# soberguo/HOIGen

Hardware: AMD Instinct MI355X
Metric: union-crop embeddings/sec ViT-B/16 bs=256 (higher is better)
Workload: dtype f16; 1 GPU; CLIP ViT-B/16 union-region encode (encode_image), 224x224 crops, batch 256 per GPU, synthetic N(0,1) crops + seeded synthetic weights (BASELINE.json configs[1]); last_block=all rows (option last_block_row0 = 0), batch_per_gpu=256, global_batch=256, parallelism=dp1

## Files before the change

### hoigen_amd/_lib.py

```python
from __future__ import annotations

import ctypes as C
import os
import subprocess
import threading
from typing import Dict, Optional

HERE = os.path.dirname(os.path.abspath(__file__))
LIB_PATH = os.environ.get("HG_LIB_PATH") or os.path.join(HERE, "csrc", "libhoigen_amd.so")
HG_MAX_SLOTS = 16
HG_F32, HG_F16 = 0, 1


class hg_tensor(C.Structure):
    _fields_ = [("ptr", C.c_void_p), ("dtype", C.c_int32)]


_BLOCK_FIELDS = ["in_proj_weight", "in_proj_bias", "out_proj_weight", "out_proj_bias", "ln_1_weight",
                 "ln_1_bias", "c_fc_weight", "c_fc_bias", "c_proj_weight", "c_proj_bias", "ln_2_weight",
                 "ln_2_bias"]


class hg_block_weights(C.Structure):
    _fields_ = [(n, hg_tensor) for n in _BLOCK_FIELDS]
# ... 81 lines not shown
    "hg_assemble_prompts": (_I, [_P, _P, _P, _P, _P, _P, _I, _I, _I, _I, _I, _P, _P]),
    "hg_l2_normalize": (_I, [_P, _P, _I, _I, _P, _P]),
    "hg_vae_loss": (_I, [_P, _P, _P, _P, _P, _I, _I, _P, _P]),
    "hg_roi_align": (_I, [_P, _P, _I, _I, _I, _P, _I, C.c_float, _I, _P, _P, _P]),
    "hg_load_cache": (_I, [_P, _I, _P]),
    "hg_cache_logits": (_I, [_P, _I, _P, _I, _P, _P]),
    "hg_preprocess_crops": (_I, [_P, _P, _I, _I, _P, _I, _I, _I, C.c_uint32, _P, _P, _P]),
    "hg_workspace_bytes": (_I, [_P, C.POINTER(C.c_uint64)]),
    "hg_set_option": (_I, [_P, C.c_char_p, _I]),
    "hg_get_option": (_I, [_P, C.c_char_p, C.POINTER(C.c_int32)]),
    "hg_test_gemm": (_I, [_P, _P, _P, _P, _P, _I, _I, _I, _I, _I, _P]),
    "hg_test_gemm_ln": (_I, [_P, _P, _P, _P, _P, _I, _I, _I, _I, _I, _P, _P, _P, _P, _P, _P, _P, _P]),
    "hg_test_attention": (_I, [_P, _P, _P, _P, _I, _I, _I, _I, _P, _P]),
    "hg_test_qkv_attn": (_I, [_P, _P, _P, _P, _P, _P, _I, _I, _I, _I, _P, _P]),
    "hg_test_gemm_hilo": (_I, [_P, _P, _P, _P, _P, _I, _I, _I, _I, _I, _P, _P, _P, _P]),
    "hg_test_image_stream": (_I, [_P, _P, _I, _P, _P, _P]),
    "hg_test_text_stream": (_I, [_P, _P, _I, _I, _I, _P, _P, _P]),
    "hg_profile_begin": (_I, [_P, _I, _I]),
    "hg_profile_end": (_I, [_P, _P, _I, C.POINTER(C.c_int32)]),
}

_lib = None
_lock = threading.RLock()
_ctxs: Dict[int, int] = {}


def build(force: bool = False) -> str:
    script = os.path.join(HERE, "csrc", "build.sh")
    if force:
        for f in os.listdir(os.path.join(HERE, "csrc")):
# ... 82 lines not shown
```

### hoigen_amd/csrc/hg_api.hip

```cpp
#include <math.h>
#include <stdarg.h>
#include <stdio.h>
#include <stdlib.h>
#include <string.h>

#include <string>
#include <vector>

#include <algorithm>
#include <mutex>

#include "../../include/hoigen_amd.h"
#include "hg_kernels.h"

using namespace hg;

namespace {

struct Buf {
    void* p = nullptr;
    size_t bytes = 0;
};

struct BlockW {
// ... 99 lines not shown
    int opt_row0 = 1;
    int opt_ln_fuse = 1;
    int opt_adapter_fuse = 1;
    int opt_adapter_fold = 1;
    int opt_stream_hilo = 1;
    int opt_qkv_attn = 1;
    int opt_qkv_attn_min_seq = 32;
    int opt_qkv_attn_gsz = 0;
    int opt_text_ln_fold = 1;
    int opt_qkv_attn_c = 1;
    int opt_vae_fused = 1;
    int opt_mlp_pair = 1;
    int opt_mlp_pair_chunk = 32;
    int opt_mlp_pair_fc_slots = 32;
    int opt_mlp_pair_fault = 0;
    int n_cu = 256;
    int32_t* pair_err = nullptr;
    int32_t* range_flag = nullptr;
    int32_t* eot_flag = nullptr;
    int32_t* eot_flag_dev = nullptr;
    int prof_kind = HG_PROF_OFF;
    std::vector<hipEvent_t> prof_ev;
    std::vector<hg_prof_rec> prof_rec;
    size_t prof_n = 0;
};

namespace {

int fail(hg_ctx* c, int code, const char* fmt, ...) {
    char tmp[512];
// ... 558 lines not shown
    half_t* const hg = gs ? (half_t*)c->hg.p : nullptr;
    half_t* a_ln = gs ? hg : h;
    auto gs_args = [&](GemmArgs& g, const float* gamma) {
        if (!gs) return;
        g.gamma = gamma;
        if (g.hl == 1 || g.hl == 2) { g.out3 = hg; g.ld3 = D; a_ln = hg; }
        else a_ln = h;
    };
    const int pair_panels = (int)rup(mlp_pair_ready_words(M), 64);
    const bool pair_on = fuse && !adapters && c->opt_mlp_pair && c->pair_err && blocks.size() > 1;
    if (pair_on) {
        int rc = ensure(c, c->pair_ready, blocks.size() * (size_t)pair_panels * 4);
        if (rc) return rc;
        HG_HIP(hipMemsetAsync(c->pair_ready.p, 0, blocks.size() * (size_t)pair_panels * 4, s));
    }
    int rln_i = 0;
    bool x_is_hilo = false;
    auto rln_args = [&](GemmArgs& g) {
        if (!hilo) return;
        g.hl = rln_i == 0 ? 1 : (rln_i == n_rln - 1 ? 3 : 2);
        g.lo = (half_t*)c->xlo.p; g.muc = muc;
        x_is_hilo = g.hl != 3;
        ++rln_i;
    };
    for (size_t i = 0; i < blocks.size(); ++i) {
        const BlockW& b = blocks[i];
        const int kcat = kmode[i];
        if (adapters && c->vit.adapters.size() > i && c->vit.adapters[i].present) {
            const AdapterW& aw = c->vit.adapters[i];
            if (kcat) {
// ... 74 lines not shown
            g.lda = D + 64; g.K = D + 64; g.W = c->vit.adapters[i].fold[ac->priors ? 0 : 1].wk_out;
        }
        if (fuse) {
            g.out2 = h; g.stats = stats; g.stats_ld = sld; g.mu = mu;
            if (hilo_c) { g.out2 = att; g.ld2 = D + 64; }
            if (!kcat || hilo_c) rln_args(g);
            gs_args(g, b.ln2_w);
            HG_HIP(gemm(c, EPI_RESID_LN_F32, g, s));
            HG_HIP(launch_finalize_stats(stats, mr, mu, M, sld, 64, s, muc, false, c->range_flag));
        } else {
            HG_HIP(gemm(c, EPI_BIAS_RESID_F32, g, s));
        }
        g = GemmArgs{};
        g.A = h; g.lda = D; g.out = fc; g.ldc = 4 * D; g.M = M; g.N = 4 * D; g.K = D;
        GemmArgs pq{};
        bool pq_built = false, paired = false;
        if (fuse) {
            g.W = b.wf_fc; g.bias = b.bf_fc; g.cs = b.cs_fc; g.mr = mr;
            if (hilo_c) { g.A = att; g.lda = D + 64; }
            if (gs) { g.A = a_ln; g.W = b.w_fc; g.cs = b.csg_fc; }
            if (pair_on && i + 1 < blocks.size()) {
                pq.A = fc; pq.lda = 4 * D; pq.W = b.w_proj; pq.bias = b.b_proj; pq.out = x; pq.ldc = D; pq.M = M; pq.N = D; pq.K = 4 * D;
                pq.out2 = h_of(i + 1); pq.ld2 = ldh_of(i + 1); pq.stats = stats; pq.stats_ld = sld; pq.mu = mu;
                rln_args(pq);
                gs_args(pq, blocks[i + 1].ln1_w);
                pq_built = true;
                if (mlp_pair_ok(g, pq, c->n_cu)) {
                    PairGateScope gate(c->device, s);
                    ProfScope ps(c, s, HG_PROF_MLP_PAIR, M, 4 * D, D);
                    HG_HIP(launch_mlp_pair(g, pq, (unsigned*)c->pair_ready.p + i * (size_t)pair_panels, c->pair_err,
                                           c->opt_mlp_pair_chunk, c->opt_mlp_pair_fc_slots, c->n_cu, s, c->opt_mlp_pair_fault));
                    paired = true;
                }
            }
            if (!paired) HG_HIP(gemm(c, EPI_LN_BIAS_QGELU_F16, g, s));
        } else {
            HG_HIP(launch_layernorm_f16(x, b.ln2_w, b.ln2_b, h, M, D, nullptr, 0, 1, s));
            g.W = b.w_fc; g.bias = b.b_fc;
            HG_HIP(gemm(c, EPI_BIAS_QGELU_F16, g, s));
        }
        g = GemmArgs{};
        g.A = fc; g.lda = 4 * D; g.W = b.w_proj; g.bias = b.b_proj; g.out = x; g.ldc = D; g.M = M; g.N = D; g.K = 4 * D;
        if (fuse && i + 1 < blocks.size()) {
            if (pq_built) {
                g = pq;
            } else {
                g.out2 = h_of(i + 1); g.ld2 = ldh_of(i + 1); g.stats = stats; g.stats_ld = sld; g.mu = mu;
                rln_args(g);
                gs_args(g, blocks[i + 1].ln1_w);
            }
            if (!paired) HG_HIP(gemm(c, EPI_RESID_LN_F32, g, s));
            HG_HIP(launch_finalize_stats(stats, mr, mu, M, sld, 64, s, muc, false, c->range_flag));
        } else {
            HG_HIP(gemm(c, EPI_BIAS_RESID_F32, g, s));
        }
        if (trace) {
            float* tr = trace + (size_t)(i + 1) * trace_stride;
            if (x_is_hilo) HG_HIP(launch_copy_rows_hilo(h, (const half_t*)c->xlo.p, muc, tr, tr_rows, tr_stride, D, s));
            else HG_HIP(launch_copy_rows(x, tr, tr_rows, tr_stride, D, s));
        }
    }
    return HG_OK;
}

int ensure_tower_ws(hg_ctx* c, int M, int D) {
    const size_t Mp = rup(M, 256);
// ... 100 lines not shown
        if (hipDeviceGetAttribute(&ncu, hipDeviceAttributeMultiprocessorCount, device) == hipSuccess && ncu > 0) c->n_cu = ncu;
        if (hipHostMalloc((void**)&c->eot_flag, 64, hipHostMallocMapped) == hipSuccess && c->eot_flag) *c->eot_flag = 0;
        else c->eot_flag = nullptr;
        if (hipMalloc((void**)&c->eot_flag_dev, 64) != hipSuccess) c->eot_flag_dev = nullptr;
        else (void)hipMemset(c->eot_flag_dev, 0, 64);
        if (hipHostMalloc((void**)&c->pair_err, 64, hipHostMallocMapped) == hipSuccess && c->pair_err) *c->pair_err = 0;
        else c->pair_err = nullptr;
        if (hipHostMalloc((void**)&c->range_flag, 64, hipHostMallocMapped) == hipSuccess && c->range_flag) *c->range_flag = 0;
        else c->range_flag = nullptr;
    }
    struct { const char* env; const char* key; } init[] = {{"HG_CHUNK_ROWS", "chunk_rows"}, {"HG_LAST_BLOCK_ROW0", "last_block_row0"},
                                                           {"HG_LN_FUSE", "ln_fuse"}, {"HG_ADAPTER_FUSE", "adapter_fuse"},
                                                           {"HG_ADAPTER_FOLD", "adapter_fold"}, {"HG_STREAM_HILO", "stream_hilo"},
                                                           {"HG_QKV_ATTN", "qkv_attn"}, {"HG_QKV_ATTN_MIN_SEQ", "qkv_attn_min_seq"},
                                                           {"HG_QKV_ATTN_GSZ", "qkv_attn_gsz"}, {"HG_QKV_ATTN_C", "qkv_attn_c"}, {"HG_TEXT_LN_FOLD", "text_ln_fold"}, {"HG_VAE_FUSED", "vae_fused"},
                                                           {"HG_MLP_PAIR", "mlp_pair"},
                                                           {"HG_MLP_PAIR_CHUNK", "mlp_pair_chunk"}, {"HG_MLP_PAIR_FC_SLOTS", "mlp_pair_fc_slots"},
                                                           {"HG_MLP_PAIR_FAULT", "mlp_pair_fault"}};
    for (auto& o : init)
        if (const char* e = getenv(o.env)) (void)hg_set_option(c, o.key, atoi(e));
    c->err.clear();
    return c;
}

int hg_set_option(hg_ctx* c, const char* key, int value) {
    if (!c || !key) return HG_ERR_INVALID;
    const std::string k(key);
    if (k == "chunk_rows") {
        if (value < 256) return fail(c, HG_ERR_INVALID, "chunk_rows must be >= 256");
        c->max_chunk_rows = value;
    } else if (k == "last_block_row0") c->opt_row0 = value != 0;
// ... 11 lines not shown
        if (value < 0 || value > 6) return fail(c, HG_ERR_INVALID, "qkv_attn_gsz must be 0 .. 6 (got %d)", value);
        c->opt_qkv_attn_gsz = value;
    } else if (k == "text_ln_fold") {
        if (value < 0 || value > 2) return fail(c, HG_ERR_INVALID, "text_ln_fold must be 0, 1 or 2 (got %d)", value);
        c->opt_text_ln_fold = value;
    } else if (k == "qkv_attn_c") {
        if (value < 0 || value > 1) return fail(c, HG_ERR_INVALID, "qkv_attn_c must be 0 or 1 (got %d)", value);
        c->opt_qkv_attn_c = value;
    }
    else if (k == "vae_fused") {
        if (value < 0 || value > 2) return fail(c, HG_ERR_INVALID, "vae_fused must be 0, 1 or 2 (got %d)", value);
        c->opt_vae_fused = value;
    } else if (k == "mlp_pair") {
        if (value < 0 || value > 1) return fail(c, HG_ERR_INVALID, "mlp_pair must be 0 or 1 (got %d)", value);
        c->opt_mlp_pair = value;
    } else if (k == "mlp_pair_chunk") {
        if (value < 1 || value > 64) return fail(c, HG_ERR_INVALID, "mlp_pair_chunk must be 1 .. 64 (got %d)", value);
        c->opt_mlp_pair_chunk = value;
    } else if (k == "mlp_pair_fc_slots") {
        if (value < 1 || value > 64) return fail(c, HG_ERR_INVALID, "mlp_pair_fc_slots must be 1 .. 64 (got %d)", value);
        c->opt_mlp_pair_fc_slots = value;
    } else if (k == "mlp_pair_fault") {
        if (value < 0 || value > 1) return fail(c, HG_ERR_INVALID, "mlp_pair_fault must be 0 or 1 (got %d)", value);
        c->opt_mlp_pair_fault = value;
    }
    else return fail(c, HG_ERR_INVALID, "unknown option '%s'", key);
    return HG_OK;
}

int hg_get_option(hg_ctx* c, const char* key, int* value) {
// ... 1 lines not shown
    const std::string k(key);
    if (k == "chunk_rows") *value = c->max_chunk_rows;
    else if (k == "last_block_row0") *value = c->opt_row0;
    else if (k == "ln_fuse") *value = c->opt_ln_fuse;
    else if (k == "adapter_fuse") *value = c->opt_adapter_fuse;
    else if (k == "adapter_fold") *value = c->opt_adapter_fold;
    else if (k == "stream_hilo") *value = c->opt_stream_hilo;
    else if (k == "stream_lo_bits") *value = 8;
    else if (k == "qkv_attn") *value = c->opt_qkv_attn;
    else if (k == "qkv_attn_min_seq") *value = c->opt_qkv_attn_min_seq;
    else if (k == "qkv_attn_gsz") *value = c->opt_qkv_attn_gsz;
    else if (k == "qkv_attn_c") *value = c->opt_qkv_attn_c;
    else if (k == "text_ln_fold") *value = c->opt_text_ln_fold;
    else if (k == "vae_fused") *value = c->opt_vae_fused;
    else if (k == "mlp_pair") *value = c->opt_mlp_pair;
    else if (k == "mlp_pair_chunk") *value = c->opt_mlp_pair_chunk;
    else if (k == "mlp_pair_fc_slots") *value = c->opt_mlp_pair_fc_slots;
    else if (k == "mlp_pair_fault") *value = c->opt_mlp_pair_fault;
    else return fail(c, HG_ERR_INVALID, "unknown option '%s'", key);
    return HG_OK;
}

void hg_destroy(hg_ctx* c) {
    if (!c) return;
    DevGuard dev_guard_(c);
    (void)hipDeviceSynchronize();
    free_all(c->vit.owned);
    free_all(c->vit.owned_adapters);
    free_all(c->text.owned);
    for (auto& v : c->vae) free_all(v.owned);
// ... 193 lines not shown
    g.A = (half_t*)c->h.p; g.lda = K; g.W = (half_t*)c->att.p; g.bias = bias; g.M = M; g.N = N; g.K = K; g.ldc = N;
    g.out = x; g.out2 = (half_t*)c->qkv.p; g.stats = (float*)c->stats.p; g.stats_ld = sld; g.mu = (const float*)c->mu.p;
    g.lo = (half_t*)c->xlo.p; g.muc = (const float*)c->muc.p;
    if (!gemm_ring2_ok(g)) return fail(c, HG_ERR_INVALID, "hg_test_gemm_hilo: shape not eligible for gemm_ring2");
    for (int i = 0; i < steps; ++i) {
        g.hl = (hilo && steps >= 2) ? (i == 0 ? 1 : (i == steps - 1 ? 3 : 2)) : 0;
        ProfScope ps(c, s, EPI_RESID_LN_F32, M, N, K);
        hipError_t e = launch_gemm_ring2(EPI_RESID_LN_F32, g, s);
        ps.finish();
        if (e != hipSuccess) return fail(c, HG_ERR_HIP, "test gemm (hi / lo) launch failed: %s", hipGetErrorString(e));
        HG_HIP(launch_finalize_stats((const float*)c->stats.p, (float*)c->mr.p, (float*)c->mu.p, M, sld, 64, s, (float*)c->muc.p));
    }
    if (out2) HG_HIP(launch_f16_to_f32((const half_t*)c->qkv.p, out2, (size_t)M * N, s));
    if (mr_out) HG_HIP(hipMemcpyAsync(mr_out, c->mr.p, (size_t)M * 2 * 4, hipMemcpyDeviceToDevice, s));
    HG_HIP(hipMemcpyAsync(mu, c->mu.p, (size_t)M * 4, hipMemcpyDeviceToDevice, s));
    return HG_OK;
}

int hg_test_attention(hg_ctx* c, const float* qkv, const float* q0, const int32_t* sel, int n_seq, int L, int heads,
                      int causal, float* out, void* stream) {
    if (!c || !qkv || !out || n_seq <= 0 || L < 1 || L > ATTN_LONG_MAX_L || heads < 1) return HG_ERR_INVALID;
    hipStream_t s = (hipStream_t)stream;
    HG_ON_DEVICE(c);
    const int D = heads * 64;
    const size_t M = (size_t)n_seq * L;
    int rc = ensure(c, c->qkv, rup(M, 256) * 3 * D * 2);
    if (!rc) rc = ensure(c, c->att, rup(M, 256) * D * 2);
    if (!rc && q0) rc = ensure(c, c->cq, rup(n_seq, 256) * (size_t)D * 2);
    if (rc) return rc;
    HG_HIP(launch_f32_to_f16(qkv, (half_t*)c->qkv.p, M * 3 * D, s));
// ... 852 lines not shown
```

### hoigen_amd/csrc/hg_gemm_ring.hip

```cpp
#include <stdio.h>
#include <stdlib.h>

#include "hg_gemm_ring_body.h"

namespace hg {

template <int MF, int EPI, bool PH2>
__global__ __launch_bounds__(512, 2) void gemm_ring(const GemmArgs p, const int tiles_n, const int n_tiles,
                                                    const unsigned a_bytes, const int mode, const int gsz) {
#if defined(__HIP_DEVICE_COMPILE__)
    const RingTileList sc(n_tiles, tiles_n, gsz);
    if (sc.n_items() <= 0) return;
    gemm_ring_body<MF, EPI, PH2>(p, a_bytes, mode, sc);
#endif
}

template <int MF, int EPI, bool PH2 = false>
static hipError_t launch_ring_t(const GemmArgs& a_in, hipStream_t s) {
    GemmArgs a = a_in;
    if (!a.ld2) a.ld2 = a.ldc;
    constexpr int BM = 64 * MF;
    constexpr int RING = 2 * (2 * MF * 4096 + 2 * 16384);
    constexpr bool LNC = (EPI == EPI_LN_BIAS_F16 || EPI == EPI_LN_BIAS_QGELU_F16);
    const int LDS = RING + a.N * 4 * (LNC ? 2 : 1) + (LNC ? BM * 8 : 0);
    if (LDS > 160 * 1024) return hipErrorInvalidValue;
    static bool attr_set_d[HG_MAX_DEVICES] = {};
    static int n_cu_d[HG_MAX_DEVICES];
    const int dev_i = current_device_index();
    bool& attr_set = attr_set_d[dev_i];
    int& n_cu = n_cu_d[dev_i];
    if (!attr_set) {
        n_cu = 256;
        hipError_t e = hipFuncSetAttribute(reinterpret_cast<const void*>(&gemm_ring<MF, EPI, PH2>),
                                           hipFuncAttributeMaxDynamicSharedMemorySize, 160 * 1024);
        if (e != hipSuccess) return e;
        int dev = 0;
        hipDeviceProp_t prop;
        if (hipGetDevice(&dev) == hipSuccess && hipGetDeviceProperties(&prop, dev) == hipSuccess)
            n_cu = prop.multiProcessorCount;
        attr_set = true;
    }
    const int tiles_m = (a.M + BM - 1) / BM, tiles_n = a.N / 256;
    const int n_tiles = tiles_m * tiles_n;
    int grid = n_tiles < n_cu ? n_tiles : n_cu;
    if (MF == 4 && n_tiles > n_cu) {
        const int rounds = (n_tiles + n_cu - 1) / n_cu;
        const int g8 = (((n_tiles + rounds - 1) / rounds) + 7) & ~7;
        if (g8 < grid) grid = g8;
// ... 3 lines not shown
    int gsz = (int)((1536 * 1024) / ((size_t)512 * a.K));
    if (gsz < 3) gsz = 3;
    if (gsz > tiles_n) gsz = tiles_n;
    {
        const int ngroups = (tiles_n + gsz - 1) / gsz;
        gsz = (tiles_n + ngroups - 1) / ngroups;
    }
#ifdef HG_STAMPS
    if (getenv("HG_STAMPS")) {
        const size_t n = (size_t)grid * 8 * 16;
        unsigned long long* d = nullptr;
        if (hipMalloc(&d, n * 8) != hipSuccess) return hipErrorOutOfMemory;
        hipMemsetAsync(d, 0, n * 8, s);
        GemmArgs b = a;
        b.dbg = d;
        hipLaunchKernelGGL((gemm_ring<MF, EPI, PH2>), dim3(grid), dim3(512), LDS, s, b, tiles_n, n_tiles, (unsigned)a_bytes, mode, gsz);
        hipStreamSynchronize(s);
        unsigned long long* h = (unsigned long long*)malloc(n * 8);
        hipMemcpy(h, d, n * 8, hipMemcpyDeviceToHost);
        static const char* names[8] = {"vmcnt", "lgkmcnt", "fetch-barrier", "MFMA", "mfma-barrier", "DMA-issue", "ds_read-issue", "epilogue"};
        for (int w = 0; w < 8; w += 4) {
            double acc[10] = {0};
            for (int blk = 0; blk < grid; ++blk)
                for (int k = 0; k < 10; ++k) acc[k] += (double)h[(size_t)(blk * 8 + w) * 16 + k];
            const double kts = acc[9] > 0 ? acc[9] : 1;
            fprintf(stderr, "[stamps] ring<%d,%d> N=%d K=%d wave %d: loop %.0f cycles/K-tile;", MF, EPI, a.N, a.K, w, acc[8] / kts);
            for (int k = 0; k < 8; ++k)
                if ((HG_STAMP_MASK >> k) & 1) fprintf(stderr, " %s %.0f", names[k], acc[k] / kts);
            fprintf(stderr, "\n");
        }
        free(h);
        hipFree(d);
        return hipGetLastError();
    }
#endif
    hipLaunchKernelGGL((gemm_ring<MF, EPI, PH2>), dim3(grid), dim3(512), LDS, s, a, tiles_n, n_tiles, (unsigned)a_bytes, mode, gsz);
    return hipGetLastError();
}

bool gemm_ring_ok(const GemmArgs& a) {
    if (a.N % 256 || a.K % 64 || a.K < 256 || a.M < 512 || a.N > 8192) return false;
    const size_t Mp = (size_t)((a.M + 255) / 256) * 256;
    if (Mp * a.lda * 2 >= (1ull << 31) || (size_t)a.N * a.K * 2 >= (1ull << 31)) return false;
    return true;
}

bool gemm_ln_ok(int epi, const GemmArgs& a) {
    if (!gemm_ring_ok(a)) return false;
    if (epi == EPI_RESID_LN_F32) return gemm_ring2_ok(a) && a.out2 && a.stats && a.mu && a.stats_ld == 4 * (a.N / 256);
    return a.cs && a.mr && a.N <= 3584;
}
// ... 22 lines not shown
        HG_RING(EPI_BIAS_QGELU_F16);
        HG_RING(EPI_BIAS_RELU_F16);
        HG_RING(EPI_BIAS_RESID_F32);
        HG_RING(EPI_BIAS_F32);
        HG_RING(EPI_PATCH_F32);
        HG_RING(EPI_BIAS_RELU_F32);
        HG_RING(EPI_SCALE_RESID_F32);
        HG_RING(EPI_LN_BIAS_F16);
        HG_RING(EPI_LN_BIAS_QGELU_F16);
        case EPI_RESID_LN_F32: return launch_ring_t<4, EPI_RESID_LN_F32, false>(a, s);
        default: return hipErrorInvalidValue;
    }
#undef HG_RING
}

}
```

### hoigen_amd/csrc/hg_gemm_ring_body.h

```cpp
#pragma once
#include <type_traits>

#include "hg_gemm_dev.h"

namespace hg {

#ifdef HG_STAMPS
#ifndef HG_STAMP_MASK
#define HG_STAMP_MASK 0xFF
#endif
#define SEG_B(k) do { if constexpr ((HG_STAMP_MASK >> (k)) & 1) t_beg = __builtin_amdgcn_s_memtime(); } while (0)
#define SEG_E(k) do { if constexpr ((HG_STAMP_MASK >> (k)) & 1) tacc[k] += __builtin_amdgcn_s_memtime() - t_beg; } while (0)
#else
#define SEG_B(k) do {} while (0)
#define SEG_E(k) do {} while (0)
#endif

template <int MF, int EPI, bool PH2, class SCHED>
__device__ __forceinline__ void gemm_ring_body(const GemmArgs& p, const unsigned a_bytes, const int mode, const SCHED& sc) {
#if defined(__HIP_DEVICE_COMPILE__)
    constexpr int BM = 64 * MF, BK = 64;
    constexpr int AH = MF * 4096, BH = 16384;
    constexpr int STAGE = 2 * AH + 2 * BH;
    constexpr int GA = MF / 2, GB = 2;
    static_assert(GA <= 2, "DMA piece helpers cover two pieces per half-tile");
    constexpr int N1 = 2 * GA + 3 * GB, N2 = 3 * GA + 2 * GB;
    constexpr bool RLN = (EPI == EPI_RESID_LN_F32);
    constexpr bool RESID = (EPI == EPI_BIAS_RESID_F32 || EPI == EPI_SCALE_RESID_F32 || RLN);
    constexpr bool F16_STORES = (EPI == EPI_BIAS_F16 || EPI == EPI_BIAS_QGELU_F16 || EPI == EPI_BIAS_RELU_F16 ||
                                 EPI == EPI_LN_BIAS_F16 || EPI == EPI_LN_BIAS_QGELU_F16);
    constexpr int E_RAW = RLN ? 8 * MF + 4 * MF + 2 * MF : (F16_STORES ? 4 * MF : 8 * MF);
    constexpr int E = E_RAW > 52 ? 52 : E_RAW;
    constexpr bool XPRE = RESID && MF == 2;
    constexpr bool LNC = (EPI == EPI_LN_BIAS_F16 || EPI == EPI_LN_BIAS_QGELU_F16);
    constexpr bool ROLL = RESID && MF == 4;
    constexpr int ROLL_W = RLN ? 6 : 8;
    constexpr int R = XPRE ? E : (ROLL ? ROLL_W + (RLN ? 1 : 0) : 0);
    constexpr bool PUB = SCHED::PUBLISH;
    static_assert(!PUB || (PH2 && (EPI == EPI_LN_BIAS_F16 || EPI == EPI_LN_BIAS_QGELU_F16)), "hand-off: two-phase loop, fp16 LayerNorm-fold epilogues");
    constexpr int BIAS_OFF = 2 * STAGE;
    const int MR_OFF = BIAS_OFF + 2 * p.N * 4;
    extern __shared__ __attribute__((aligned(16))) char smem[];
#ifdef HG_STAMPS
    unsigned long long tacc[8] = {0, 0, 0, 0, 0, 0, 0, 0}, t_beg = 0, t_all = 0;
#endif
    const int tid = sc.thread_id(), lane = tid & 63;
    const int wave = __builtin_amdgcn_readfirstlane(tid >> 6);
    const int wm = wave >> 2, wn = wave & 3;
    const int nk = p.K / BK;

    const int bid = blockIdx.x;
    const int n_items = sc.n_items();
// ... 186 lines not shown
    int g = 0;
    bool prev_full = false;
    int tm_prev = 0;
    (void)tm_prev;
    for (int r = 0; r < n_items; ++r) {
        int tm, tn, kb_r, ke_r;
        item_get(r, tm, tn, kb_r, ke_r);
        const int klen = nk;
        const int m0 = tm * BM, n0 = tn * 256;
        const bool post_ok = prev_full;
        prev_full = m0 + BM <= p.M;
        zero_acc();
        f32x4 xres[XPRE ? 2 : 1][XPRE ? 2 : 1][XPRE ? MF : 1][XPRE ? 2 : 1];
        f32x4 xw[ROLL ? ROLL_W : 1];
        float muw[RLN ? 2 : 1];
        auto chunk_row = [&](int rg) {
            int m = m0 + (rg / MF) * (BM / 2) + wm * MF * 16 + (rg % MF) * 16 + (lane & 15);
            return m < p.M ? m : p.M - 1;
        };
        auto chunk_load = [&](int c) {
            const int rg = c >> 2, hb = (c >> 1) & 1, g2 = c & 1;
            const int n = n0 + hb * 128 + wn * 32 + g2 * 16 + 4 * (lane >> 4);
            return *reinterpret_cast<const f32x4*>(reinterpret_cast<const float*>(p.out) + (size_t)chunk_row(rg) * p.ldc + n);
        };
        auto ph2_ktile = [&](auto KIND_T) {
            constexpr int KINDX = decltype(KIND_T)::value;
            constexpr int KIND = KINDX >= 4 ? 0 : KINDX;
            const int buf = (g & 1) * STAGE;
            const bool post = post_ok;
            const bool more = KIND < 2 || r + 1 < n_items;
// ... 72 lines not shown
            ph2_ktile(K1{});
            if constexpr (PUB) {
                ph2_ktile(std::integral_constant<int, 4>{});
                ph2_ktile(std::integral_constant<int, 5>{});
            }
            for (int kt = PUB ? 3 : 1; kt < klen - 2; ++kt) {
                ph2_ktile(K0{});
            }
            ph2_ktile(K2{});
            ph2_ktile(K3{});
        } else {
        for (int kt = 0; kt < klen; ++kt, ++g) {
            const int buf = (g & 1) * STAGE;
            const bool more = g + 2 < S;
            const bool post = post_ok;
            const bool xl = (XPRE || ROLL) && kt == klen - 1;
            read_A(0, buf);
            read_W(I0{}, buf);
            if constexpr (LNC) {
                if (kt == klen - 2 && lane < BM / 16)
                    __builtin_amdgcn_raw_ptr_buffer_load_lds(rsM, (HG_LDS void*)(smem + MR_OFF + wave * BM), 16, lane * 16,
                                                             (m0 + wave * (BM / 8)) * 8, 0, 0);
            }
            if (g + 1 < S) issue_A(1, 0, GA);
            if constexpr (ROLL) {
                if (xl) {
#pragma unroll
                    for (int c = 0; c < ROLL_W; ++c) xw[c] = chunk_load(c);
                    if constexpr (RLN) muw[0] = p.mu[chunk_row(0)];
                }
            }
            if constexpr (XPRE) {
                if (xl) {
#pragma unroll
                    for (int ha = 0; ha < 2; ++ha)
#pragma unroll
                        for (int f = 0; f < MF; ++f) {
                            int m = m0 + ha * (BM / 2) + wm * MF * 16 + f * 16 + (lane & 15);
                            m = m < p.M ? m : p.M - 1;
#pragma unroll
                            for (int hb = 0; hb < 2; ++hb)
#pragma unroll
                                for (int g2 = 0; g2 < 2; ++g2) {
                                    const int n = n0 + hb * 128 + wn * 32 + g2 * 16 + 4 * (lane >> 4);
                                    xres[ha][hb][f][g2] = *reinterpret_cast<const f32x4*>(
// ... 89 lines not shown
                    u32x4 st0, st1;
#pragma unroll
                    for (int j = 0; j < 4; ++j) {
                        const unsigned send = low ? d[4 + j] : d[j];
                        const unsigned recv = (unsigned)__builtin_amdgcn_update_dpp(0, (int)send, 0x128, 0xF, 0xF, false);
                        st0[j] = low ? d[j] : recv;
                        st1[j] = low ? recv : d[4 + j];
                    }
                    const int row0 = mb + (r16 & 7);
                    if (INTERIOR || row0 < p.M) *reinterpret_cast<u32x4*>(colp + (size_t)row0 * p.ldc) = st0;
                    if (INTERIOR || row0 + 8 < p.M) *reinterpret_cast<u32x4*>(colp + (size_t)(row0 + 8) * p.ldc) = st1;
                }
            };
            if (m0 + BM <= p.M) f16_epilogue(std::true_type{});
            else f16_epilogue(std::false_type{});
        } else if constexpr (ROLL) {
            const int q = lane >> 4;
            typedef unsigned u32x2 __attribute__((ext_vector_type(2)));
            typedef unsigned u32x4 __attribute__((ext_vector_type(4)));
#pragma unroll
            for (int rg = 0; rg < 2 * MF; ++rg) {
                const int ha = rg / MF, f = rg % MF;
                const int m = m0 + ha * (BM / 2) + wm * MF * 16 + f * 16 + (lane & 15);
                f32x4 v[2][2];
                float mu_r = 0.f;
                if constexpr (RLN) {
                    mu_r = muw[rg & 1];
                    if (rg + 1 < 2 * MF) muw[(rg + 1) & 1] = p.mu[chunk_row(rg + 1)];
                }
#pragma unroll
// ... 103 lines not shown
```

### hoigen_amd/csrc/hg_kernels.h

```cpp
#pragma once
#include <hip/hip_runtime.h>
#include <stdint.h>

#include "hg_common.h"

namespace hg {

enum Epilogue : int {
    EPI_BIAS_F16 = 0,
    EPI_BIAS_QGELU_F16 = 1,
    EPI_BIAS_RELU_F16 = 2,
    EPI_BIAS_RESID_F32 = 3,
    EPI_BIAS_F32 = 4,
    EPI_PATCH_F32 = 5,
    EPI_BIAS_RELU_F32 = 6,
    EPI_SCALE_RESID_F32 = 7,
    EPI_LN_BIAS_F16 = 8,
    EPI_LN_BIAS_QGELU_F16 = 9,
    EPI_RESID_LN_F32 = 10,
    EPI_MU_BIAS_RELU_F32 = 11,
    EPI_SCALE_RESID_LN_F32 = 12
};

#ifndef HG_LO_SCALE
// ... 24 lines not shown
    const float* muc = nullptr;
    const float* gamma = nullptr;
    half_t* out3 = nullptr;
    int ld3 = 0;
};
inline size_t gemm_lo_bytes(int M, int N) { return (size_t)((M + 127) / 128) * (N / 256) * 65536; }

hipError_t launch_gemm(int epi, const GemmArgs& a, hipStream_t s);
double gemm_flops(const GemmArgs& a);
bool gemm_ring_ok(const GemmArgs& a);
hipError_t launch_gemm_ring(int epi, const GemmArgs& a, hipStream_t s);
bool gemm_ring2_ok(const GemmArgs& a);
bool gemm_ln_ok(int epi, const GemmArgs& a);
hipError_t launch_gemm_ring2(int epi, const GemmArgs& a, hipStream_t s);
hipError_t launch_gemm_simple(int epi, const GemmArgs& a, hipStream_t s);
bool mlp_pair_ok(const GemmArgs& fc, const GemmArgs& proj, int n_cu);
size_t mlp_pair_ready_words(int M);
hipError_t launch_mlp_pair(const GemmArgs& fc, const GemmArgs& proj, unsigned* ready, int* err, int ch, int fc_slots, int n_cu, hipStream_t s,
                           int grid_short = 0);
bool gemm_duo_ok(int epi, const GemmArgs& a);
hipError_t launch_gemm_duo(int epi, const GemmArgs& a, hipStream_t s);

static constexpr int ATTN_MAX_L_RESIDENT = 224;
static constexpr int ATTN_LONG_MAX_L = 640;
hipError_t launch_attention(const half_t* qkv, half_t* out, int n_seq, int L, int heads, bool causal,
                            hipStream_t s, int ldo = 0, bool pack = true);
hipError_t launch_attention_row0(const half_t* qkv, const half_t* q0, const int32_t* sel, half_t* out, int n_seq, int L,
                                 int heads, bool causal, hipStream_t s);
hipError_t launch_attention_long(const half_t* qkv, half_t* out, int n_seq, int L, int heads, bool causal, hipStream_t s, int ldo);
hipError_t launch_attention_long_row0(const half_t* qkv, const half_t* q0, const int32_t* sel, half_t* out, int n_seq, int L,
// ... 135 lines not shown
```

### include/hoigen_amd.h

```cpp
#ifndef HOIGEN_AMD_H
#define HOIGEN_AMD_H

#include <stdint.h>

#ifdef __cplusplus
extern "C" {
#endif

typedef struct hg_ctx hg_ctx;

typedef enum {
    HG_OK = 0,
    HG_ERR_INVALID = -1,
    HG_ERR_HIP = -2,
    HG_ERR_NOT_LOADED = -3,
    HG_ERR_OOM = -4
} hg_status;

typedef enum { HG_F32 = 0, HG_F16 = 1 } hg_dtype;

typedef struct {
    const void* ptr;
    int32_t dtype;
} hg_tensor;
// ... 131 lines not shown
#define HG_PROF_MLP_PAIR 103
typedef struct {
    int32_t kind;
    int32_t M, N, K;
    float ms;
} hg_prof_rec;
int hg_profile_begin(hg_ctx*, int kind, int max_launches);
int hg_profile_end(hg_ctx*, hg_prof_rec* recs, int max_recs, int32_t* n_recs);
int hg_test_gemm(hg_ctx*, const float* a, const float* w, const float* bias, float* out, int M, int N, int K,
                 int epi, int kernel, void* stream);
int hg_test_gemm_ln(hg_ctx*, const float* a, const float* w, const float* bias, float* out, int M, int N, int K, int epi,
                    int kernel, const float* cs, const float* mr, const float* mu, const float* scale, float* out2,
                    float* mr_out, float* mu_out, void* stream);
int hg_test_gemm_hilo(hg_ctx*, const float* a, const float* w, const float* bias, float* x, int M, int N, int K, int steps,
                      int hilo, float* mu, float* out2, float* mr_out, void* stream);
int hg_test_attention(hg_ctx*, const float* qkv, const float* q0, const int32_t* sel, int n_seq, int L, int heads,
                      int causal, float* out, void* stream);

int hg_test_qkv_attn(hg_ctx*, const float* a, const float* w, const float* bias, const float* cs, const float* mr, int n_seq,
                     int L, int heads, int fused, float* out, void* stream);

int hg_test_image_stream(hg_ctx*, const float* x_nchw, int B, float* out, float* trace, void* stream);
int hg_test_text_stream(hg_ctx*, const int32_t* ids, int T, int L, int trunc, float* out, float* trace, void* stream);

#ifdef __cplusplus
}
#endif
#endif
```

Measured before the change: 24760 crops/s.

## Add wide 256-row c_proj residual-LN GEMM path with hi/lo residual streaming

Adds a new path for the MLP c_proj GEMM with residual plus LayerNorm-stats epilogue. It uses 256-row tiles over a number of rows sized to fill whole rounds of CUs, then runs the ragged remainder through the existing ring GEMM. The epilogue is extended to read and write the residual as an fp16 hi plus bf8 lo split, so the full fp32 residual stream need not be loaded or stored. It is on by default and takes precedence over the mlp_pair fused kernel. This trades the cross-GEMM pairing and adds a second launch for the tail rows.

```diff
diff --git a/hoigen_amd/_lib.py b/hoigen_amd/_lib.py
--- a/hoigen_amd/_lib.py
+++ b/hoigen_amd/_lib.py
@@ -119,6 +119,7 @@
     "hg_test_attention": (_I, [_P, _P, _P, _P, _I, _I, _I, _I, _P, _P]),
     "hg_test_qkv_attn": (_I, [_P, _P, _P, _P, _P, _P, _I, _I, _I, _I, _P, _P]),
     "hg_test_gemm_hilo": (_I, [_P, _P, _P, _P, _P, _I, _I, _I, _I, _I, _P, _P, _P, _P]),
+    "hg_test_gemm_wide": (_I, [_P, _P, _P, _P, _P, _P, _P, _P, _P, _P, _I, _I, _I, _I, _I, _P]),
     "hg_test_image_stream": (_I, [_P, _P, _I, _P, _P, _P]),
     "hg_test_text_stream": (_I, [_P, _P, _I, _I, _I, _P, _P, _P]),
     "hg_profile_begin": (_I, [_P, _I, _I]),
diff --git a/hoigen_amd/csrc/hg_api.hip b/hoigen_amd/csrc/hg_api.hip
--- a/hoigen_amd/csrc/hg_api.hip
+++ b/hoigen_amd/csrc/hg_api.hip
@@ -137,6 +137,7 @@
     int opt_mlp_pair_chunk = 32;
     int opt_mlp_pair_fc_slots = 32;
     int opt_mlp_pair_fault = 0;
+    int opt_cproj_wide = 1;
     int n_cu = 256;
     int32_t* pair_err = nullptr;
     int32_t* range_flag = nullptr;
@@ -725,6 +726,7 @@
         if (rc) return rc;
         HG_HIP(hipMemsetAsync(c->pair_ready.p, 0, blocks.size() * (size_t)pair_panels * 4, s));
     }
+    const bool wide_on = fuse && !adapters && !causal && !gs && c->opt_cproj_wide && blocks.size() > 1;
     int rln_i = 0;
     bool x_is_hilo = false;
     auto rln_args = [&](GemmArgs& g) {
@@ -829,18 +831,19 @@
         g = GemmArgs{};
         g.A = h; g.lda = D; g.out = fc; g.ldc = 4 * D; g.M = M; g.N = 4 * D; g.K = D;
         GemmArgs pq{};
-        bool pq_built = false, paired = false;
+        bool pq_built = false, paired = false, wide = false;
         if (fuse) {
             g.W = b.wf_fc; g.bias = b.bf_fc; g.cs = b.cs_fc; g.mr = mr;
             if (hilo_c) { g.A = att; g.lda = D + 64; }
             if (gs) { g.A = a_ln; g.W = b.w_fc; g.cs = b.csg_fc; }
-            if (pair_on && i + 1 < blocks.size()) {
+            if ((pair_on || wide_on) && i + 1 < blocks.size()) {
                 pq.A = fc; pq.lda = 4 * D; pq.W = b.w_proj; pq.bias = b.b_proj; pq.out = x; pq.ldc = D; pq.M = M; pq.N = D; pq.K = 4 * D;
                 pq.out2 = h_of(i + 1); pq.ld2 = ldh_of(i + 1); pq.stats = stats; pq.stats_ld = sld; pq.mu = mu;
                 rln_args(pq);
                 gs_args(pq, blocks[i + 1].ln1_w);
                 pq_built = true;
-                if (mlp_pair_ok(g, pq, c->n_cu)) {
+                wide = wide_on && gemm_resid_wide_ok(pq);
+                if (!wide && pair_on && mlp_pair_ok(g, pq, c->n_cu)) {
                     PairGateScope gate(c->device, s);
                     ProfScope ps(c, s, HG_PROF_MLP_PAIR, M, 4 * D, D);
                     HG_HIP(launch_mlp_pair(g, pq, (unsigned*)c->pair_ready.p + i * (size_t)pair_panels, c->pair_err,
@@ -864,7 +867,12 @@
                 rln_args(g);
                 gs_args(g, blocks[i + 1].ln1_w);
             }
-            if (!paired) HG_HIP(gemm(c, EPI_RESID_LN_F32, g, s));
+            if (wide) {
+                ProfScope ps(c, s, EPI_RESID_LN_F32, g.M, g.N, g.K);
+                HG_HIP(launch_gemm_resid_wide(g, s));
+            } else if (!paired) {
+                HG_HIP(gemm(c, EPI_RESID_LN_F32, g, s));
+            }
             HG_HIP(launch_finalize_stats(stats, mr, mu, M, sld, 64, s, muc, false, c->range_flag));
         } else {
             HG_HIP(gemm(c, EPI_BIAS_RESID_F32, g, s));
@@ -995,7 +1003,7 @@
                                                            {"HG_ADAPTER_FOLD", "adapter_fold"}, {"HG_STREAM_HILO", "stream_hilo"},
                                                            {"HG_QKV_ATTN", "qkv_attn"}, {"HG_QKV_ATTN_MIN_SEQ", "qkv_attn_min_seq"},
                                                            {"HG_QKV_ATTN_GSZ", "qkv_attn_gsz"}, {"HG_QKV_ATTN_C", "qkv_attn_c"}, {"HG_TEXT_LN_FOLD", "text_ln_fold"}, {"HG_VAE_FUSED", "vae_fused"},
-                                                           {"HG_MLP_PAIR", "mlp_pair"},
+                                                           {"HG_MLP_PAIR", "mlp_pair"}, {"HG_CPROJ_WIDE", "cproj_wide"},
                                                            {"HG_MLP_PAIR_CHUNK", "mlp_pair_chunk"}, {"HG_MLP_PAIR_FC_SLOTS", "mlp_pair_fc_slots"},
                                                            {"HG_MLP_PAIR_FAULT", "mlp_pair_fault"}};
     for (auto& o : init)
@@ -1037,6 +1045,9 @@
     } else if (k == "mlp_pair") {
         if (value < 0 || value > 1) return fail(c, HG_ERR_INVALID, "mlp_pair must be 0 or 1 (got %d)", value);
         c->opt_mlp_pair = value;
+    } else if (k == "cproj_wide") {
+        if (value < 0 || value > 1) return fail(c, HG_ERR_INVALID, "cproj_wide must be 0 or 1 (got %d)", value);
+        c->opt_cproj_wide = value;
     } else if (k == "mlp_pair_chunk") {
         if (value < 1 || value > 64) return fail(c, HG_ERR_INVALID, "mlp_pair_chunk must be 1 .. 64 (got %d)", value);
         c->opt_mlp_pair_chunk = value;
@@ -1068,6 +1079,7 @@
     else if (k == "text_ln_fold") *value = c->opt_text_ln_fold;
     else if (k == "vae_fused") *value = c->opt_vae_fused;
     else if (k == "mlp_pair") *value = c->opt_mlp_pair;
+    else if (k == "cproj_wide") *value = c->opt_cproj_wide;
     else if (k == "mlp_pair_chunk") *value = c->opt_mlp_pair_chunk;
     else if (k == "mlp_pair_fc_slots") *value = c->opt_mlp_pair_fc_slots;
     else if (k == "mlp_pair_fault") *value = c->opt_mlp_pair_fault;
@@ -1291,6 +1303,30 @@
     if (out2) HG_HIP(launch_f16_to_f32((const half_t*)c->qkv.p, out2, (size_t)M * N, s));
     if (mr_out) HG_HIP(hipMemcpyAsync(mr_out, c->mr.p, (size_t)M * 2 * 4, hipMemcpyDeviceToDevice, s));
     HG_HIP(hipMemcpyAsync(mu, c->mu.p, (size_t)M * 4, hipMemcpyDeviceToDevice, s));
+    return HG_OK;
+}
+
+int hg_test_gemm_wide(hg_ctx* c, const float* a, const float* w, const float* bias, float* x, void* hi, void* lo, const float* mu,
+                      const float* muc, float* stats, int M, int N, int K, int hl, int kernel, void* stream) {
+    if (!c || !a || !w || !x || !hi || !mu || !stats || M <= 0 || hl < 0 || hl > 3 || (hl && (!lo || !muc))) return HG_ERR_INVALID;
+    if (N % 256) return fail(c, HG_ERR_INVALID, "hg_test_gemm_wide: N must be a multiple of 256");
+    hipStream_t s = (hipStream_t)stream;
+    HG_ON_DEVICE(c);
+    int rc = ensure(c, c->h, rup(M, 256) * K * 2);
+    if (!rc) rc = ensure(c, c->att, (size_t)N * K * 2);
+    if (rc) return rc;
+    HG_HIP(launch_f32_to_f16(a, (half_t*)c->h.p, (size_t)M * K, s));
+    HG_HIP(launch_f32_to_f16(w, (half_t*)c->att.p, (size_t)N * K, s));
+    GemmArgs g{};
+    g.A = (half_t*)c->h.p; g.lda = K; g.W = (half_t*)c->att.p; g.bias = bias; g.M = M; g.N = N; g.K = K; g.ldc = N;
+    g.out = x; g.out2 = (half_t*)hi; g.ld2 = N; g.stats = stats; g.stats_ld = 4 * (N / 256); g.mu = mu;
+    g.hl = hl; g.lo = (half_t*)lo; g.muc = muc;
+    if (kernel ? !gemm_resid_wide_ok(g) : !gemm_ln_ok(EPI_RESID_LN_F32, g))
+        return fail(c, HG_ERR_INVALID, "hg_test_gemm_wide: shape not eligible (M = %d, N = %d, K = %d, kernel %d)", M, N, K, kernel);
+    ProfScope ps(c, s, EPI_RESID_LN_F32, M, N, K);
+    const hipError_t e = kernel ? launch_gemm_resid_wide(g, s) : launch_gemm_ring2(EPI_RESID_LN_F32, g, s);
+    ps.finish();
+    if (e != hipSuccess) return fail(c, HG_ERR_HIP, "test gemm (wide) launch failed: %s", hipGetErrorString(e));
     return HG_OK;
 }
 
diff --git a/hoigen_amd/csrc/hg_gemm_ring.hip b/hoigen_amd/csrc/hg_gemm_ring.hip
--- a/hoigen_amd/csrc/hg_gemm_ring.hip
+++ b/hoigen_amd/csrc/hg_gemm_ring.hip
@@ -15,8 +15,25 @@
 #endif
 }
 
-template <int MF, int EPI, bool PH2 = false>
+template <int HL>
+__global__ __launch_bounds__(512, 2) void gemm_ring_wide(const GemmArgs p, const int tiles_n, const int n_tiles,
+                                                         const unsigned a_bytes, const int mode, const int gsz) {
+#if defined(__HIP_DEVICE_COMPILE__)
+    const RingTileList sc(n_tiles, tiles_n, gsz);
+    if (sc.n_items() <= 0) return;
+    gemm_ring_body<4, EPI_RESID_LN_F32, false, RingTileList, HL>(p, a_bytes, mode, sc);
+#endif
+}
+
+template <int MF, int EPI, bool PH2, int HL>
+static constexpr auto ring_kernel() {
+    if constexpr (HL != 0) return &gemm_ring_wide<HL>;
+    else return &gemm_ring<MF, EPI, PH2>;
+}
+
+template <int MF, int EPI, bool PH2 = false, int HL = 0>
 static hipError_t launch_ring_t(const GemmArgs& a_in, hipStream_t s) {
+    constexpr auto kern = ring_kernel<MF, EPI, PH2, HL>();
     GemmArgs a = a_in;
     if (!a.ld2) a.ld2 = a.ldc;
     constexpr int BM = 64 * MF;
@@ -31,7 +48,7 @@
     int& n_cu = n_cu_d[dev_i];
     if (!attr_set) {
         n_cu = 256;
-        hipError_t e = hipFuncSetAttribute(reinterpret_cast<const void*>(&gemm_ring<MF, EPI, PH2>),
+        hipError_t e = hipFuncSetAttribute(reinterpret_cast<const void*>(kern),
                                            hipFuncAttributeMaxDynamicSharedMemorySize, 160 * 1024);
         if (e != hipSuccess) return e;
         int dev = 0;
@@ -65,7 +82,7 @@
         hipMemsetAsync(d, 0, n * 8, s);
         GemmArgs b = a;
         b.dbg = d;
-        hipLaunchKernelGGL((gemm_ring<MF, EPI, PH2>), dim3(grid), dim3(512), LDS, s, b, tiles_n, n_tiles, (unsigned)a_bytes, mode, gsz);
+        hipLaunchKernelGGL(kern, dim3(grid), dim3(512), LDS, s, b, tiles_n, n_tiles, (unsigned)a_bytes, mode, gsz);
         hipStreamSynchronize(s);
         unsigned long long* h = (unsigned long long*)malloc(n * 8);
         hipMemcpy(h, d, n * 8, hipMemcpyDeviceToHost);
@@ -85,7 +102,7 @@
         return hipGetLastError();
     }
 #endif
-    hipLaunchKernelGGL((gemm_ring<MF, EPI, PH2>), dim3(grid), dim3(512), LDS, s, a, tiles_n, n_tiles, (unsigned)a_bytes, mode, gsz);
+    hipLaunchKernelGGL(kern, dim3(grid), dim3(512), LDS, s, a, tiles_n, n_tiles, (unsigned)a_bytes, mode, gsz);
     return hipGetLastError();
 }
 
@@ -138,4 +155,54 @@
 #undef HG_RING
 }
 
-}
+static int device_cu_count() {
+    static int n_cu_d[HG_MAX_DEVICES] = {};
+    int& n_cu = n_cu_d[current_device_index()];
+    if (!n_cu) {
+        int dev = 0;
+        hipDeviceProp_t prop;
+        n_cu = (hipGetDevice(&dev) == hipSuccess && hipGetDeviceProperties(&prop, dev) == hipSuccess) ? prop.multiProcessorCount : 256;
+    }
+    return n_cu;
+}
+
+int gemm_resid_wide_rows(const GemmArgs& a) {
+    if (a.N % 256 || a.M < 256) return 0;
+    const int tiles_n = a.N / 256, n_cu = device_cu_count();
+    const int rounds = (int)(((long long)(a.M / 256) * tiles_n) / n_cu);
+    return (rounds * n_cu / tiles_n) * 256;
+}
+
+bool gemm_resid_wide_ok(const GemmArgs& a) {
+    return gemm_ln_ok(EPI_RESID_LN_F32, a) && !a.gamma && a.hl >= 0 && a.hl <= 3 && (!a.ld2 || a.ld2 % 8 == 0) &&
+           (!a.hl || (a.lo && ((a.hl != 2 && a.hl != 3) || a.muc))) && gemm_resid_wide_rows(a) > 0;
+}
+
+hipError_t launch_gemm_resid_wide(const GemmArgs& a_in, hipStream_t s) {
+    if (!gemm_resid_wide_ok(a_in)) return hipErrorInvalidValue;
+    GemmArgs a = a_in;
+    if (!a.ld2) a.ld2 = a.ldc;
+    const int rows = gemm_resid_wide_rows(a);
+    GemmArgs big = a;
+    big.M = rows;
+    hipError_t e;
+    switch (a.hl) {
+        case 0: e = launch_ring_t<4, EPI_RESID_LN_F32, false>(big, s); break;
+        case 1: e = launch_ring_t<4, EPI_RESID_LN_F32, false, 1>(big, s); break;
+        case 2: e = launch_ring_t<4, EPI_RESID_LN_F32, false, 2>(big, s); break;
+        default: e = launch_ring_t<4, EPI_RESID_LN_F32, false, 3>(big, s); break;
+    }
+    if (e != hipSuccess || rows >= a.M) return e;
+    GemmArgs rest = a;
+    rest.M = a.M - rows;
+    rest.A = a.A + (size_t)rows * a.lda;
+    rest.out = reinterpret_cast<float*>(a.out) + (size_t)rows * a.ldc;
+    rest.out2 = a.out2 + (size_t)rows * a.ld2;
+    rest.stats = a.stats + (size_t)rows * a.stats_ld * 2;
+    rest.mu = a.mu + rows;
+    if (a.muc) rest.muc = a.muc + rows;
+    if (a.lo) rest.lo = a.lo + (size_t)(rows / 128) * (a.N / 256) * 16384;
+    return launch_gemm_ring2(EPI_RESID_LN_F32, rest, s);
+}
+
+}
diff --git a/hoigen_amd/csrc/hg_gemm_ring_body.h b/hoigen_amd/csrc/hg_gemm_ring_body.h
--- a/hoigen_amd/csrc/hg_gemm_ring_body.h
+++ b/hoigen_amd/csrc/hg_gemm_ring_body.h
@@ -16,7 +16,7 @@
 #define SEG_E(k) do {} while (0)
 #endif
 
-template <int MF, int EPI, bool PH2, class SCHED>
+template <int MF, int EPI, bool PH2, class SCHED, int HL = 0>
 __device__ __forceinline__ void gemm_ring_body(const GemmArgs& p, const unsigned a_bytes, const int mode, const SCHED& sc) {
 #if defined(__HIP_DEVICE_COMPILE__)
     constexpr int BM = 64 * MF, BK = 64;
@@ -29,13 +29,17 @@
     constexpr bool RESID = (EPI == EPI_BIAS_RESID_F32 || EPI == EPI_SCALE_RESID_F32 || RLN);
     constexpr bool F16_STORES = (EPI == EPI_BIAS_F16 || EPI == EPI_BIAS_QGELU_F16 || EPI == EPI_BIAS_RELU_F16 ||
                                  EPI == EPI_LN_BIAS_F16 || EPI == EPI_LN_BIAS_QGELU_F16);
-    constexpr int E_RAW = RLN ? 8 * MF + 4 * MF + 2 * MF : (F16_STORES ? 4 * MF : 8 * MF);
+    static_assert(HL == 0 || (EPI == EPI_RESID_LN_F32 && MF == 4), "hi / lo stream: EPI_RESID_LN_F32 on 256-row tiles");
+    static_assert(HL == 0 || !PH2, "hi / lo stream: four-phase K loop");
+    constexpr bool IN_HL = (HL == 2 || HL == 3), OUT_HL = (HL == 1 || HL == 2);
+    constexpr int E_RAW = RLN ? (OUT_HL ? 4 * MF + 4 * MF + 2 * MF : 8 * MF + 4 * MF + 2 * MF) : (F16_STORES ? 4 * MF : 8 * MF);
     constexpr int E = E_RAW > 52 ? 52 : E_RAW;
     constexpr bool XPRE = RESID && MF == 2;
     constexpr bool LNC = (EPI == EPI_LN_BIAS_F16 || EPI == EPI_LN_BIAS_QGELU_F16);
-    constexpr bool ROLL = RESID && MF == 4;
-    constexpr int ROLL_W = RLN ? 6 : 8;
-    constexpr int R = XPRE ? E : (ROLL ? ROLL_W + (RLN ? 1 : 0) : 0);
+    constexpr bool ROLL = RESID && MF == 4 && !IN_HL;
+    constexpr int ROLL_W = RLN ? (HL == 1 ? 4 : 6) : 8;
+    constexpr int HL_NU = 2, HL_UL = 12;
+    constexpr int R = XPRE ? E : (ROLL ? ROLL_W + (RLN ? 1 : 0) : (IN_HL ? HL_UL : 0));
     constexpr bool PUB = SCHED::PUBLISH;
     static_assert(!PUB || (PH2 && (EPI == EPI_LN_BIAS_F16 || EPI == EPI_LN_BIAS_QGELU_F16)), "hand-off: two-phase loop, fp16 LayerNorm-fold epilogues");
     constexpr int BIAS_OFF = 2 * STAGE;
@@ -252,6 +256,40 @@
         f32x4 xres[XPRE ? 2 : 1][XPRE ? 2 : 1][XPRE ? MF : 1][XPRE ? 2 : 1];
         f32x4 xw[ROLL ? ROLL_W : 1];
         float muw[RLN ? 2 : 1];
+        typedef unsigned u32x4_hl __attribute__((ext_vector_type(4)));
+        typedef unsigned u32x2_hl __attribute__((ext_vector_type(2)));
+        u32x4_hl xhi[IN_HL ? HL_NU : 1][IN_HL ? 2 : 1][IN_HL ? 2 : 1];
+        u32x2_hl xlo[IN_HL ? HL_NU : 1][IN_HL ? 2 : 1][IN_HL ? 2 : 1];
+        float muv[IN_HL ? HL_NU : 1][IN_HL ? 2 : 1], mucv[IN_HL ? HL_NU : 1][IN_HL ? 2 : 1];
+        auto tm_here = [&]() {
+            int t = tm;
+            asm volatile("" : "+s"(t));
+            return t;
+        };
+        auto lo_ptr = [&](int tm_, int u, int hb, int g2) {
+            const unsigned lo_lane = (unsigned)((wn * 8 + wm * 4) * 256 + lane * 4);
+            const unsigned t = (unsigned)(((2 * tm_ + (u >> 1)) * (p.N / 256) + tn) * 16384 + (u & 1) * 8192);
+            return p.lo + (t + lo_lane + (unsigned)((hb * 2 + g2) * 256));
+        };
+        auto unit_row = [&](int tm_, int u) { return tm_ * BM + (u >> 1) * (BM / 2) + wm * MF * 16 + (u & 1) * 32 + (lane & 15); };
+        auto hl_load = [&](auto U_T) {
+            constexpr int u = decltype(U_T)::value, sl = u % HL_NU;
+            const int tm_ = tm_here();
+            const int mp = unit_row(tm_, u) + (((lane >> 4) & 1) ? 16 : 0);
+#pragma unroll
+            for (int hb = 0; hb < 2; ++hb)
+#pragma unroll
+                for (int g2 = 0; g2 < 2; ++g2) {
+                    xhi[sl][hb][g2] = *reinterpret_cast<const u32x4_hl*>(
+                        p.out2 + (size_t)mp * p.ld2 + n0 + hb * 128 + wn * 32 + g2 * 16 + 4 * ((lane >> 4) & ~1));
+                    xlo[sl][hb][g2] = *reinterpret_cast<const u32x2_hl*>(lo_ptr(tm_, u, hb, g2));
+                }
+#pragma unroll
+            for (int f2 = 0; f2 < 2; ++f2) {
+                muv[sl][f2] = p.mu[unit_row(tm_, u) + f2 * 16];
+                mucv[sl][f2] = p.muc[unit_row(tm_, u) + f2 * 16];
+            }
+        };
         auto chunk_row = [&](int rg) {
             int m = m0 + (rg / MF) * (BM / 2) + wm * MF * 16 + (rg % MF) * 16 + (lane & 15);
             return m < p.M ? m : p.M - 1;
@@ -354,7 +392,7 @@
             const int buf = (g & 1) * STAGE;
             const bool more = g + 2 < S;
             const bool post = post_ok;
-            const bool xl = (XPRE || ROLL) && kt == klen - 1;
+            const bool xl = (XPRE || ROLL || IN_HL) && kt == klen - 1;
             read_A(0, buf);
             read_W(I0{}, buf);
             if constexpr (LNC) {
@@ -369,6 +407,9 @@
                     for (int c = 0; c < ROLL_W; ++c) xw[c] = chunk_load(c);
                     if constexpr (RLN) muw[0] = p.mu[chunk_row(0)];
                 }
+            }
+            if constexpr (IN_HL) {
+                if (xl) hl_load(std::integral_constant<int, 0>{});
             }
             if constexpr (XPRE) {
                 if (xl) {
@@ -488,6 +529,145 @@
             };
             if (m0 + BM <= p.M) f16_epilogue(std::true_type{});
             else f16_epilogue(std::false_type{});
+        } else if constexpr (HL != 0) {
+            const int q = lane >> 4;
+            typedef unsigned u32x2 __attribute__((ext_vector_type(2)));
+            typedef unsigned u32x4 __attribute__((ext_vector_type(4)));
+            typedef float f32x2 __attribute__((ext_vector_type(2)));
+            if constexpr (IN_HL) {
+                hl_load(std::integral_constant<int, 1>{});
+                if constexpr (HL_NU > 2) hl_load(std::integral_constant<int, 2>{});
+                __builtin_amdgcn_sched_barrier(0);
+            }
+            auto unit = [&](auto U_T) {
+                constexpr int u = decltype(U_T)::value, ha = u >> 1, fp = u & 1, sl = IN_HL ? u % HL_NU : 0;
+                half4 h16[2][2][2];
+                unsigned l8[OUT_HL ? 2 : 1][OUT_HL ? 2 : 1][OUT_HL ? 2 : 1];
+                const int tm_ = tm_here();
+                half4 hin[IN_HL ? 2 : 1][IN_HL ? 2 : 1][IN_HL ? 2 : 1];
+                f32x4 lin[IN_HL ? 2 : 1][IN_HL ? 2 : 1][IN_HL ? 2 : 1];
+                if constexpr (IN_HL) {
+#pragma unroll
+                    for (int hb = 0; hb < 2; ++hb)
+#pragma unroll
+                        for (int g2 = 0; g2 < 2; ++g2) {
+                            const u32x4_hl o = xhi[sl][hb][g2];
+                            const u32x2_hl l = xlo[sl][hb][g2];
+                            const auto s0 = __builtin_amdgcn_permlane16_swap(o[0], o[2], false, false);
+                            const auto s1 = __builtin_amdgcn_permlane16_swap(o[1], o[3], false, false);
+                            hin[0][hb][g2] = __builtin_bit_cast(half4, u32x2{(unsigned)s0[0], (unsigned)s1[0]});
+                            hin[1][hb][g2] = __builtin_bit_cast(half4, u32x2{(unsigned)s0[1], (unsigned)s1[1]});
+#pragma unroll
+                            for (int f2 = 0; f2 < 2; ++f2) {
+                                const auto a = __builtin_amdgcn_cvt_pk_f32_bf8((int)l[f2], false);
+                                const auto b = __builtin_amdgcn_cvt_pk_f32_bf8((int)l[f2], true);
+                                lin[f2][hb][g2] = f32x4{a[0], a[1], b[0], b[1]};
+                            }
+                        }
+                }
+#pragma unroll
+                for (int f2 = 0; f2 < 2; ++f2) {
+                    const int f = 2 * fp + f2, rg = ha * MF + f;
+                    const int m = unit_row(tm_, u) + f2 * 16;
+                    float mu_r, muc_r = 0.f;
+                    if constexpr (IN_HL) {
+                        mu_r = muv[sl][f2];
+                        muc_r = mucv[sl][f2];
+                    } else {
+                        mu_r = muw[rg & 1];
+                        if (rg + 1 < 2 * MF) muw[(rg + 1) & 1] = p.mu[chunk_row(rg + 1)];
+                    }
+                    (void)muc_r;
+                    f32x4 v[2][2];
+                    float sum = 0.f;
+#pragma unroll
+                    for (int hb = 0; hb < 2; ++hb)
+#pragma unroll
+                        for (int g2 = 0; g2 < 2; ++g2) {
+                            const int n = n0 + hb * 128 + wn * 32 + g2 * 16 + 4 * q;
+                            f32x4 xin;
+                            if constexpr (IN_HL) {
+                                const f32x2 mc2 = {muc_r, muc_r};
+#pragma unroll
+                                for (int e2 = 0; e2 < 2; ++e2) {
+                                    const half2v h2 = {hin[f2][hb][g2][2 * e2], hin[f2][hb][g2][2 * e2 + 1]};
+                                    const f32x2 ls2 = {1.0f / HG_LO_SCALE, 1.0f / HG_LO_SCALE};
+                                    const f32x2 x2 = f32x2{lin[f2][hb][g2][2 * e2], lin[f2][hb][g2][2 * e2 + 1]} * ls2 +
+                                                     (mc2 + __builtin_convertvector(h2, f32x2));
+                                    xin[2 * e2] = x2[0];
+                                    xin[2 * e2 + 1] = x2[1];
+                                }
+                            } else {
+                                const int c = (rg * 2 + hb) * 2 + g2;
+                                xin = xw[c % ROLL_W];
+                                if (c + ROLL_W < 8 * MF) xw[c % ROLL_W] = chunk_load(c + ROLL_W);
+                            }
+                            v[hb][g2] = xin + (acc[ha][hb][f][g2] + *reinterpret_cast<const f32x4*>(smem + BIAS_OFF + n * 4));
+                            sum += (v[hb][g2][0] + v[hb][g2][1]) + (v[hb][g2][2] + v[hb][g2][3]);
+                            if constexpr (!OUT_HL)
+                                *reinterpret_cast<f32x4*>(reinterpret_cast<float*>(p.out) + (size_t)m * p.ldc + n) = v[hb][g2];
+                            const f32x2 mu2 = {mu_r, mu_r};
+                            float rem[4];
+#pragma unroll
+                            for (int e2 = 0; e2 < 2; ++e2) {
+                                const f32x2 d = f32x2{v[hb][g2][2 * e2], v[hb][g2][2 * e2 + 1]} - mu2;
+                                const half2v hh = __builtin_convertvector(d, half2v);
+                                h16[f2][hb][g2][2 * e2] = hh[0];
+                                h16[f2][hb][g2][2 * e2 + 1] = hh[1];
+                                if constexpr (OUT_HL) {
+                                    const f32x2 r2 = d - __builtin_convertvector(hh, f32x2);
+                                    const f32x2 rs = r2 * f32x2{HG_LO_SCALE, HG_LO_SCALE};
+                                    rem[2 * e2] = rs[0];
+                                    rem[2 * e2 + 1] = rs[1];
+                                }
+                            }
+                            if constexpr (OUT_HL) {
+                                int w8 = __builtin_amdgcn_cvt_pk_bf8_f32(rem[0], rem[1], 0, false);
+                                w8 = __builtin_amdgcn_cvt_pk_bf8_f32(rem[2], rem[3], w8, true);
+                                l8[f2][hb][g2] = (unsigned)w8;
+                            }
+                            if constexpr (!IN_HL) __builtin_amdgcn_sched_barrier(0);
+                        }
+                    sum = sum_rows(sum);
+                    const float gm = sum * (1.0f / 64.0f);
+                    float m2 = 0.f;
+#pragma unroll
+                    for (int hb = 0; hb < 2; ++hb)
+#pragma unroll
+                        for (int g2 = 0; g2 < 2; ++g2)
+#pragma unroll
+                            for (int e2 = 0; e2 < 2; ++e2) {
+                                const f32x2 d = f32x2{v[hb][g2][2 * e2], v[hb][g2][2 * e2 + 1]} - f32x2{gm, gm};
+                                m2 = fmaf(d[0], d[0], m2);
+                                m2 = fmaf(d[1], d[1], m2);
+                            }
+                    m2 = sum_rows(m2);
+                    if (q == 0)
+                        *reinterpret_cast<f32x2*>(p.stats + ((size_t)m * p.stats_ld + (n0 / 256) * 4 + wn) * 2) = f32x2{sum, m2};
+                }
+                const int mp = unit_row(tm_, u) + ((q & 1) ? 16 : 0);
+#pragma unroll
+                for (int hb = 0; hb < 2; ++hb)
+#pragma unroll
+                    for (int g2 = 0; g2 < 2; ++g2) {
+                        const int nb = n0 + hb * 128 + wn * 32 + g2 * 16;
+                        const u32x2 ux = __builtin_bit_cast(u32x2, h16[0][hb][g2]), uy = __builtin_bit_cast(u32x2, h16[1][hb][g2]);
+                        const auto s0 = __builtin_amdgcn_permlane16_swap(ux[0], uy[0], false, false);
+                        const auto s1 = __builtin_amdgcn_permlane16_swap(ux[1], uy[1], false, false);
+                        const u32x4 o = {s0[0], s1[0], s0[1], s1[1]};
+                        *reinterpret_cast<u32x4*>(p.out2 + (size_t)mp * p.ld2 + nb + 4 * (q & ~1)) = o;
+                        if constexpr (OUT_HL) *reinterpret_cast<u32x2*>(lo_ptr(tm_, u, hb, g2)) = u32x2{l8[0][hb][g2], l8[1][hb][g2]};
+                    }
+                if constexpr (IN_HL && u + HL_NU < 4) {
+                    __builtin_amdgcn_sched_barrier(0);
+                    hl_load(std::integral_constant<int, u + HL_NU>{});
+                    __builtin_amdgcn_sched_barrier(0);
+                }
+            };
+            unit(std::integral_constant<int, 0>{});
+            unit(std::integral_constant<int, 1>{});
+            unit(std::integral_constant<int, 2>{});
+            unit(std::integral_constant<int, 3>{});
         } else if constexpr (ROLL) {
             const int q = lane >> 4;
             typedef unsigned u32x2 __attribute__((ext_vector_type(2)));
diff --git a/hoigen_amd/csrc/hg_kernels.h b/hoigen_amd/csrc/hg_kernels.h
--- a/hoigen_amd/csrc/hg_kernels.h
+++ b/hoigen_amd/csrc/hg_kernels.h
@@ -62,6 +62,9 @@
 bool gemm_ln_ok(int epi, const GemmArgs& a);
 hipError_t launch_gemm_ring2(int epi, const GemmArgs& a, hipStream_t s);
 hipError_t launch_gemm_simple(int epi, const GemmArgs& a, hipStream_t s);
+int gemm_resid_wide_rows(const GemmArgs& a);
+bool gemm_resid_wide_ok(const GemmArgs& a);
+hipError_t launch_gemm_resid_wide(const GemmArgs& a, hipStream_t s);
 bool mlp_pair_ok(const GemmArgs& fc, const GemmArgs& proj, int n_cu);
 size_t mlp_pair_ready_words(int M);
 hipError_t launch_mlp_pair(const GemmArgs& fc, const GemmArgs& proj, unsigned* ready, int* err, int ch, int fc_slots, int n_cu, hipStream_t s,
diff --git a/include/hoigen_amd.h b/include/hoigen_amd.h
--- a/include/hoigen_amd.h
+++ b/include/hoigen_amd.h
@@ -169,6 +169,8 @@
                     float* mr_out, float* mu_out, void* stream);
 int hg_test_gemm_hilo(hg_ctx*, const float* a, const float* w, const float* bias, float* x, int M, int N, int K, int steps,
                       int hilo, float* mu, float* out2, float* mr_out, void* stream);
+int hg_test_gemm_wide(hg_ctx*, const float* a, const float* w, const float* bias, float* x, void* hi, void* lo, const float* mu,
+                      const float* muc, float* stats, int M, int N, int K, int hl, int kernel, void* stream);
 int hg_test_attention(hg_ctx*, const float* qkv, const float* q0, const int32_t* sel, int n_seq, int L, int heads,
                       int causal, float* out, void* stream);
 
```

Result: no change. 24790 crops/s, median of 2 (+0.1%).
